# uthree/tinyvc

Hardware: AMD Instinct MI355X
Metric: audio-samples/sec (16 kHz) end-to-end VC (higher is better)
Workload: dtype f32 (fp32 in / out / accumulate; channel contractions as two-term fp16 splits on v_mfma_f32_32x32x16_f16: 22-bit significands, three part-products per fp32 product)

## Files before the change

### tinyvc_amd/csrc/decoder.hip

```cpp
#include "conv3s.h"
#include "conv_s2.h"
#include "film_s2.h"
#include "gemm_s2.h"
#include "small_kernels.h"
#include "tvc_common.h"

namespace tvc {


__device__ __forceinline__ float div24k(float x) {
    const float r = 1.0f / 24000.0f;
    const float q0 = __fmul_rn(x, r);
    return fmaf(fmaf(-q0, 24000.0f, x), r, q0);
}

__device__ __forceinline__ double wave_incl_scan(double v, int lane) {
#pragma unroll
    for (int o = 1; o < 64; o <<= 1) {
        double u = __shfl_up(v, o);
        if (lane >= o) v += u;
    }
    return v;
}

// ... 191 lines not shown
    hipStream_t sh = s;
    if (fk) {
        sh = fk->side;
        TVC_HIP(ctx, hipStreamWaitEvent(sh, fk->amps_ready, 0));
    } else {
        TVC_CHECK(run_harm_sums(ctx, s, f0, csum, B, T));
    }
    hipLaunchKernelGGL(harm_synth_kernel, dim3((Tg + 3) / 4, NB), dim3(256), 0, sh, f0, amps, csum, source, T, scale_size, scale_amp, rg);
    TVC_CHECK(run_amax_rows(ctx, sh, amps, B, kHarm, T, smax));
    TVC_CHECK(run_noise_ifft(ctx, s, kern, angle, seed, frames, B, T, ctx->rag && angle));
    hipLaunchKernelGGL(noise_ola_kernel, dim3(grid_for((long)Tg * kHop / 4, 256, NB >= 32 ? 16 : 512 / NB), NB), dim3(256), 0, s, frames, source, B, T, smax, rg);
    return launch_check(ctx, "dsp");
}

static int plain_conv(tvc_ctx* ctx, hipStream_t s, const PackedW& w, const float* x, int B, int Cin, int len, int dil, float* y, const BfpSlots& bfp, int lin = 0,
                      float lscale = 0.f) {
    int rc = 0;
    if ((lin > 0 ? conv_s2_try<true>(&rc, ctx, s, w, x, B, Cin, len, dil, y, bfp, lin, lscale) : conv_s2_try<false>(&rc, ctx, s, w, x, B, Cin, len, dil, y, bfp)))
        return rc;
    if (lin > 0)
        return conv3s_launch<true, C3EpiBias<false>, false, true>(ctx, s, w, x, B, Cin, len, dil, C3EpiBias<false>{y, w.bias, nullptr, w.M, len}, bfp, nullptr, nullptr,
                                                                   nullptr, 0, lin, lscale);
    return conv3s_launch<true>(ctx, s, w, x, B, Cin, len, dil, C3EpiBias<false>{y, w.bias, nullptr, w.M, len}, bfp);
}

static int film_conv(tvc_ctx* ctx, hipStream_t s, const PackedW& w, const PackedW& fw, const FilmU& fu, const float* h, const float* cond, int B, int C, int len, int dil,
                     float* out, const float* bsc, const float* bsh, const float* res, int res_lin, float res_scale, const BfpSlots& bfp) {
    int rc = 0;
    if (rag_min_len(ctx, len) >= FS2::BN && film_s2_try(&rc, ctx, s, fu, h, cond, B, C, len, dil, out, res, res_lin, res_scale, bfp)) return rc;
    return conv3s_launch<true, C3EpiFilmFused, true>(ctx, s, w, h, B, C, len, dil, C3EpiFilmFused{out, w.bias, bsc, bsh, res, C, len, res_lin, res_scale}, bfp, &fw, &fw,
                                                     cond, C);
}

static int conv_film_half(tvc_ctx* ctx, hipStream_t s, const PackedW& ca, const PackedW& cb, const PackedW& fw, const FilmU& fu, const float* x, int lin, float lscale,
                          int da, int db, float* h, const float* cond, int B, int C, int len, float* out, const float* bsc, const float* bsh, const float* res,
                          int res_lin, float res_scale, const float* ma_in, float* mh, const float* mcond, float* mout) {
    const bool pre = rag_min_len(ctx, len) >= FS2::BN && fu.img && fu.C == C && fu.hb_w > 0.f && C % 96 == 0 && C <= 384 && ma_in && mcond && res && db >= 1 && db <= FS2::MAXD &&
                     (long)C * len * 4 < (1L << 32) && (res_lin <= 0 || (long)C * res_lin * 4 < (1L << 32));
    if (pre) {
        int rc = 0;
        const BfpSlots in{ma_in, nullptr, nullptr};
        const bool ok = lin > 0 ? conv_s2_try<true, true>(&rc, ctx, s, ca, x, B, C, len, da, h, in, lin, lscale, fu.hb_w, fu.hb_b)
                                : conv_s2_try<false, true>(&rc, ctx, s, ca, x, B, C, len, da, h, in, 0, 0.f, fu.hb_w, fu.hb_b);
        if (ok) {
            TVC_CHECK(rc);
            if (!film_s2_try(&rc, ctx, s, fu, h, cond, B, C, len, db, out, res, res_lin, res_scale, BfpSlots{ma_in, mcond, mout}, true, fu.hb_w, fu.hb_b))
                return fail(ctx, TVC_ERR_STATE, "filter_net: the FiLM conv refused the pre-split operand its producer wrote");
            return rc;
        }
    }
    TVC_CHECK(plain_conv(ctx, s, ca, x, B, C, len, da, h, BfpSlots{ma_in, nullptr, mh}, lin, lscale));
    return film_conv(ctx, s, cb, fw, fu, h, cond, B, C, len, db, out, bsc, bsh, res, res_lin, res_scale, BfpSlots{mh, mcond, mout});
}

static __global__ void g8_to_planar_kernel(const float* __restrict__ x, float* __restrict__ y, long B, long l, int C) {
    const long n = B * C * l;
    for (long i = blockIdx.x * (long)blockDim.x + threadIdx.x; i < n; i += (long)gridDim.x * blockDim.x) {
        const long t = i % l, bc = i / l, c = bc % C, b = bc / C;
        y[i] = x[((b * (C / 8) + c / 8) * l + t) * 8 + (c & 7)];
    }
}

static int filter_input_gemm(tvc_ctx* ctx, hipStream_t s, const float* content, const float* f0, float* x, int B, int T, const float* cmax) {
    EpiSumCond ep{x, ctx->flt_content_in.bias, nullptr, f0, nullptr, nullptr, ctx->flt_f_w, ctx->flt_f_b, 384, T, B * T};
    int rc = 0;
    if (!gemm_s2_try(&rc, ctx, s, ctx->flt_content_in, content, B, kSslDim, T, 0, ep, cmax)) rc = gemm_s_launch<2, 4, 2>(ctx, s, ctx->flt_content_in, content, B, kSslDim, T, 0, ep, cmax);
    return rc;
}

int run_filter(tvc_ctx* ctx, hipStream_t s, Ws& ws, const float* content, const float* f0,
               const float* energy, const float* source, float* wave, int B, int T, const FilterTaps* taps, const float* cmax, const float* smax, float* zeroed_slots, bool x_slot_set,
               float* x_pre, bool x_pre_filled) {
    const long L = (long)T * kHop;
    static const int ch[5] = {384, 192, 96, 48, 24};
    const long len_dn[5] = {L, L / 5, L / 20, L / 80, L / 240};
    float* skip[5];
    for (int i = 0; i < 5; ++i) skip[i] = ws.get<float>((size_t)B * ch[4 - i] * len_dn[i]);
    float* x = x_pre ? x_pre : ws.get<float>((size_t)B * ch[0] * T);
    float* xi_pre[5] = {nullptr, nullptr, nullptr, nullptr, nullptr};
    for (int i = 1; i <= 4; ++i) xi_pre[i] = ws.get<float>((size_t)B * ctx->downs[i - 1].cin * len_dn[i]);
// ... 52 lines not shown
                                                                 BfpSlots{mh2, mxi, mout}, &d.res, nullptr, xi, d.cin)));
            }
        }
        ws.release(mk);
    }
    float* xlev[5];
    {
        long l = T;
        for (int i = 0; i < 5; ++i) {
            l *= ctx->ups[i].factor;
            xlev[i] = ws.get<float>((size_t)B * ctx->ups[i].cout * l);
        }
    }
    long len = T;
    const float* mx_in = slot(S_X);
    for (int i = 0; i < 5; ++i) {
        const UpW& u = ctx->ups[i];
        const int lin = (int)len;
        len *= u.factor;
        const int lo = (int)len, C = u.cin, nc = B * lo;
        const float* cond = skip[4 - i];
        const float* mcond = slot(S_SKIP0 + 4 - i);
        size_t mk = ws.mark();
        float* xu = ws.get<float>((size_t)B * C * lo);
        float* h = ws.get<float>((size_t)B * C * lo);
        float* x1 = ws.get<float>((size_t)B * C * lo);
        if (!ws.dry && C == 24) {
            ProfScope ps(ctx, s, ws, "filter.up4+out");
            TVC_CHECK(run_up24_split(ctx, s, u, x, cond, ctx->down0_bw, ctx->down0_bb, x1, wave, B, lo, mx_in, smax, slot(S_UX1 + i)));
        } else if (!ws.dry) {
            static const char* names[4] = {"filter.up0", "filter.up1", "filter.up2", "filter.up3"};
            ProfScope ps(ctx, s, ws, names[i]);
            const float lscale = (float)(1.0 / (double)u.factor);
            for (int half = 0; half < 2; ++half) {
                const PackedW& ca = half ? u.c3 : u.c1;
                const PackedW& cb = half ? u.c4 : u.c2;
                const PackedW& fw = half ? u.film2 : u.film1;
                const float* bsc = fw.bias;
                const float* bsh = fw.bias + C;
                const int da = half ? 9 : 1, db = half ? 27 : 3;
                float* xout = half ? xu : x1;
                const float* ma_in = half ? slot(S_UX1 + i) : mx_in;
                float* mh = slot((half ? S_UHB : S_UHA) + i);
                float* mout = slot((half ? S_UXU : S_UX1) + i);
                if (C == 48) {
                    if (half == 0) {
                        TVC_CHECK(run_conv48_pair(ctx, s, ca, cb, x, lin, lscale, &fw, bsc, bsh, cond, xout, B, lo, da, db, ma_in, mcond, mout));
                    } else {
                        TVC_CHECK(run_conv48s(ctx, s, ca, x1, nullptr, nullptr, nullptr, nullptr, nullptr, h, B, lo, da, ma_in, nullptr, mh));
                        TVC_CHECK(run_conv48s(ctx, s, cb, h, &fw, bsc, bsh, cond, x1, nullptr, B, lo, db, mh, mcond, slot(S_LEV + i), &u.c5, xlev[i]));
                    }
                } else if (half == 0) {
                    TVC_CHECK(conv_film_half(ctx, s, ca, cb, fw, u.fu1, x, lin, lscale, da, db, h, cond, B, C, lo, xout, bsc, bsh, x, lin, lscale, ma_in, mh, mcond, mout));
                } else {
                    TVC_CHECK(conv_film_half(ctx, s, ca, cb, fw, u.fu2, x1, 0, 0.f, da, db, h, cond, B, C, lo, xout, bsc, bsh, x1, 0, 0.f, ma_in, mh, mcond, mout));
                }
            }
            if (C != 48) {
                EpiBias<ACT_NONE, false> ep{xlev[i], u.c5.bias, nullptr, u.cout, lo, nc, (long)u.cout * lo, 0, slot(S_LEV + i), slot(S_UXU + i), u.c5_bw, u.c5_bb, NB};
                if (u.cout == 48) {
                    EpiBiasG8 eg{xlev[i], u.c5.bias, u.cout, lo, nc, slot(S_LEV + i), slot(S_UXU + i), u.c5_bw, u.c5_bb, NB};
                    TVC_CHECK((gemm_s_launch<2, 4, 2>(ctx, s, u.c5, xu, B, C, lo, 0, eg, slot(S_UXU + i))));
                } else if (u.c5.MT6 % 3 == 0) TVC_CHECK((gemm_s_launch<3, 4, 1>(ctx, s, u.c5, xu, B, C, lo, 0, ep, slot(S_UXU + i))));
                else TVC_CHECK((gemm_s_launch<2, 4, 2>(ctx, s, u.c5, xu, B, C, lo, 0, ep, slot(S_UXU + i))));
            }
        }
        ws.release(mk);
        x = xlev[i];
        mx_in = slot(S_LEV + i);
    }
    if (!ws.dry && taps) {
        for (int i = 1; i < 5; ++i)
            if (taps->skips[i] && i == 1)
                hipLaunchKernelGGL(g8_to_planar_kernel, dim3(grid_for((long)B * 48 * len_dn[1])), dim3(256), 0, s, skip[1], taps->skips[1], (long)B, len_dn[1], 48);
            else if (taps->skips[i])
                TVC_HIP(ctx, hipMemcpyAsync(taps->skips[i], skip[i], (size_t)B * ch[4 - i] * len_dn[i] * sizeof(float), hipMemcpyDeviceToDevice, s));
        long l = T;
        for (int i = 0; i < 4; ++i) {
            l *= ctx->ups[i].factor;
            if (taps->ups[i] && ctx->ups[i].cout <= 48)
                hipLaunchKernelGGL(g8_to_planar_kernel, dim3(grid_for((long)B * ctx->ups[i].cout * l)), dim3(256), 0, s, xlev[i], taps->ups[i], (long)B, l, ctx->ups[i].cout);
            else if (taps->ups[i])
                TVC_HIP(ctx, hipMemcpyAsync(taps->ups[i], xlev[i], (size_t)B * ctx->ups[i].cout * l * sizeof(float), hipMemcpyDeviceToDevice, s));
        }
    }
    return ws.dry ? 0 : launch_check(ctx, "filter_net");
}

int run_decoder(tvc_ctx* ctx, hipStream_t s, Ws& ws, const float* content, const float* f0,
                const float* energy, const float* angle, uint64_t seed, float* wave, float* amps_out,
                float* kernel_out, float* source_out, int B, int T, const float* content_bound, const float* energy_bound,
// ... 49 lines not shown
```

### tinyvc_amd/csrc/film_s2.h

```cpp
#pragma once
#include "conv_s2.h"
#include "split_fp16.h"

namespace tvc {


struct FilmS2Args {
    const uint4* img;
    const float* tab;
    const float* x;
    const float* cond;
    int C, len, dil;
    float* y;
    const float* res;
    int res_lin;
    float res_scale;
    int tiles_per_utt, ntiles, mblocks;
    const float* amax_x;
    const float* amax_c;
    float* amax_y;
    const uint4* xpre;
    float pre_w, pre_b;
    RagDev rag;
};

template <int NWV_>
struct FS2T {
    static constexpr int MTB = 3, MW = 1, WM = MTB / MW, NWV = NWV_, WN = 1, NW = MW * NWV, NTHR = NW * 64, BN = NWV * WN * 32, MAXD = 27, XROW = BN + 2 * MAXD;
    static constexpr int A_CONV = 3 * MTB * 2, A_PIECES = A_CONV + 2 * MTB * 2, A_PER = (A_PIECES + NW - 1) / NW;
    static constexpr int XS = (2 * XROW + NTHR - 1) / NTHR;
    static constexpr int A_U4 = A_PIECES * 64, X_U4 = 2 * 2 * XROW, C_U4 = 2 * 2 * BN, BUF_U4 = A_U4 + X_U4 + C_U4;
    static constexpr int lds_bytes = 2 * BUF_U4 * 16 + 6 * 384 * 4 + 64;
    static_assert(2 * BN <= NTHR, "one cond item per thread");
};
using FS2 = FS2T<8>;

__device__ __forceinline__ void split8u(const float (&v)[8], uint4& p1, uint4& p2) {
    unsigned o1[4], o2[4];
#pragma unroll
    for (int j = 0; j < 4; ++j) split2<false>(v[2 * j], v[2 * j + 1], o1[j], o2[j]);
    p1 = make_uint4(o1[0], o1[1], o1[2], o1[3]);
    p2 = make_uint4(o2[0], o2[1], o2[2], o2[3]);
}

template <bool XPRE, bool RAG = false, int NWV_ = 8>
__global__ __launch_bounds__(FS2T<NWV_>::NTHR) __attribute__((amdgpu_waves_per_eu(2))) void film_s2_kernel(FilmS2Args a) {
    using TL = FS2T<NWV_>;
    constexpr int MTB = TL::MTB, WM = TL::WM, NWV = TL::NWV, WN = TL::WN, NW = TL::NW, BN = TL::BN, XROW = TL::XROW, A_PER = TL::A_PER, XS = TL::XS;
    extern __shared__ __attribute__((aligned(16))) uint4 smem_fs[];
    float* Tb = reinterpret_cast<float*>(smem_fs + 2 * TL::BUF_U4);
    float* red = Tb + 6 * 384;
    const int tid = threadIdx.x, lane = tid & 63;
    const int wave = __builtin_amdgcn_readfirstlane(tid >> 6);
    const int l31 = lane & 31, lh = lane >> 5;
    const int wm = wave / NWV, wn = wave - wm * NWV;
    const int C = a.C, nslab = C / 16, rs = a.len, dil = a.dil;
    const int rf = a.res_lin > 0 ? rs / a.res_lin : 1;
    const int xw = BN + 2 * dil, nitems = 2 * xw;

    for (int i = tid; i < 6 * C; i += TL::NTHR) {
        const int r = i / C;
        Tb[r * 384 + (i - r * C)] = a.tab[i];
    }

    int tfirst, tlast;
    tile_range(a.ntiles, tfirst, tlast);
    if (tfirst >= tlast) return;
    auto coords = [&](int v, int& mb, int& b, int& t0, int& len, int& off) __attribute__((always_inline)) {
        const int nt = v / a.mblocks;
        mb = v - nt * a.mblocks;
        const RagTile rt = rag_tile<RAG>(a.rag, nt, a.tiles_per_utt, rs, b);
        b = rt.b;
        t0 = rt.tin * BN;
        len = rt.len;
        off = rt.off;
    };

    u32x4 ar[A_PER];
    float xr[XPRE ? 1 : XS][8], cr[8];
    uint4 xq[XPRE ? XS : 1][2];
    auto item_of = [&](int t_, int k, int& g, int& c) __attribute__((always_inline)) {
        int item = t_ + k * TL::NTHR;
        item = item < nitems ? item : item - nitems;
        g = item / xw;
        c = item - g * xw;
    };
    int xdst[XS];
#pragma unroll
    for (int k = 0; k < XS; ++k) {
        int g, c;
        item_of(tid, k, g, c);
        xdst[k] = g * XROW + c;
    }
    const int cg = tid >= BN ? 1 : 0, cc = tid - cg * BN;
    const int cdst = cg * BN + cc;
// ... 124 lines not shown
        }
    };
    auto film_mul = [&](int buf) __attribute__((always_inline)) {
        const uint4* Ab = smem_fs + buf * TL::BUF_U4 + (TL::A_CONV + wm * WM * 2) * 64 + lane;
        const uint4* Cb = smem_fs + buf * TL::BUF_U4 + TL::A_U4 + TL::X_U4 + lh * BN + wn * WN * 32 + l31;
        f16x8 bf[WN][2];
#pragma unroll
        for (int j = 0; j < WN; ++j)
#pragma unroll
            for (int p = 0; p < 2; ++p) bf[j][p] = __builtin_bit_cast(f16x8, Cb[p * 2 * BN + j * 32]);
#pragma unroll
        for (int i = 0; i < WM; ++i) {
            f16x8 af[2], ag[2];
#pragma unroll
            for (int p = 0; p < 2; ++p) af[p] = __builtin_bit_cast(f16x8, Ab[(i * 2 + p) * 64]);
#pragma unroll
            for (int p = 0; p < 2; ++p) ag[p] = __builtin_bit_cast(f16x8, Ab[((MTB + i) * 2 + p) * 64]);
#pragma unroll
            for (int j = 0; j < WN; ++j) {
                sc[i][j] = TVC_MFMA16(af[1], bf[j][0], sc[i][j]);
                sh[i][j] = TVC_MFMA16(ag[1], bf[j][0], sh[i][j]);
            }
#pragma unroll
            for (int j = 0; j < WN; ++j) {
                sc[i][j] = TVC_MFMA16(af[0], bf[j][1], sc[i][j]);
                sh[i][j] = TVC_MFMA16(ag[0], bf[j][1], sh[i][j]);
            }
#pragma unroll
            for (int j = 0; j < WN; ++j) {
                sc[i][j] = TVC_MFMA16(af[0], bf[j][0], sc[i][j]);
                sh[i][j] = TVC_MFMA16(ag[0], bf[j][0], sh[i][j]);
            }
        }
    };

    int cv = tfirst, cs = 0, cmb, cb = 0, ct0, len, coff;
    coords(cv, cmb, cb, ct0, len, coff);
    float mx_run = 0.f;
    int flush_b = -1;

    issue_load();
    advance_load();
    lstore(0);
    issue_load();
    advance_load();
    slab_barrier();
    int buf = 0;
    while (true) {
        tap_mul(buf, 0);
        lstore(buf ^ 1);
        issue_load();
        tap_mul(buf, 1);
        tap_mul(buf, 2);
        film_mul(buf);
        advance_load();
        if (++cs == nslab) {
            cs = 0;
            int el = lane;
            asm volatile("" : "+v"(el));
            const int e31 = el & 31, eh = el >> 5;
            const float ix = norm_from_amax(XPRE ? presplit_bound(a.pre_w, a.pre_b, a.amax_x, cb) : sload_f32(a.amax_x + cb)).inv, ic_ = norm_from_amax(sload_f32(a.amax_c + cb)).inv;
#pragma unroll
            for (int i = 0; i < WM; ++i) {
            const int row0 = (cmb * MTB + wm * WM + i) * 32;
            const float kc = Tb[FilmU::TAB_SCALE * 384 + row0] * ix, ks = Tb[FilmU::TAB_SSC * 384 + row0] * ic_, kh = Tb[FilmU::TAB_SSH * 384 + row0] * ic_;
#pragma unroll
            for (int g = 0; g < 4; ++g) {
                const int rr = row0 + 8 * g + 4 * eh;
                const float4 b0 = *reinterpret_cast<const float4*>(Tb + FilmU::TAB_BIAS * 384 + rr);
                const float4 b1 = *reinterpret_cast<const float4*>(Tb + FilmU::TAB_BSC * 384 + rr);
                const float4 b2 = *reinterpret_cast<const float4*>(Tb + FilmU::TAB_BSH * 384 + rr);
                const float bm[4] = {b0.x, b0.y, b0.z, b0.w}, bs[4] = {b1.x, b1.y, b1.z, b1.w}, bh[4] = {b2.x, b2.y, b2.z, b2.w};
#pragma unroll
                for (int q = 0; q < 4; ++q)
#pragma unroll
                    for (int j = 0; j < WN; ++j) {
                        const int r = 4 * g + q;
                        const float h = fmaf(hi[i][j][r], kc, bm[q]), s = fmaf(sc[i][j][r], ks, bs[q]), t = fmaf(sh[i][j][r], kh, bh[q]);
                        hi[i][j][r] = __fadd_rn(__fmul_rn(h, s), t);
                        sc[i][j][r] = 0.f;
                        sh[i][j][r] = 0.f;
                    }
            }
            float* yb = RAG ? a.y + (long)row0 * rs + coff : a.y + ((long)cb * C + row0) * rs;
#pragma unroll
            for (int j = 0; j < WN; ++j) {
                const int t = ct0 + (wn * WN + j) * 32 + e31;
                const bool live = t < len;
                const int tc = live ? t : len - 1;
                const unsigned off = 4u * (unsigned)(4 * eh * rs + tc);
                if (a.res_lin > 0) {
                    const Lerp lc = lerp_coord(tc, a.res_scale, RAG ? len / rf : a.res_lin);
                    const float* rb = RAG ? a.res + (long)row0 * a.res_lin + coff / rf : a.res + ((long)cb * C + row0) * a.res_lin;
                    const unsigned o0 = 4u * (unsigned)(4 * eh * a.res_lin + lc.i0), o1 = 4u * (unsigned)(4 * eh * a.res_lin + lc.i1);
#pragma unroll
                    for (int h8 = 0; h8 < 2; ++h8) {
                        float x0[8], x1[8];
#pragma unroll
                        for (int r = 0; r < 8; ++r) {
                            const float* rr = rb + (long)(16 * h8 + (r & 3) + 8 * (r >> 2)) * a.res_lin;
                            x0[r] = ldg_so(rr, o0);
                            x1[r] = ldg_so(rr, o1);
                        }
#pragma unroll
                        for (int r = 0; r < 8; ++r) hi[i][j][8 * h8 + r] = __fadd_rn(hi[i][j][8 * h8 + r], lerp_eval(lc, x0[r], x1[r]));
                    }
                } else {
                    const float* rb = RAG ? a.res + (long)row0 * rs + coff : a.res + ((long)cb * C + row0) * rs;
                    float rv[16];
#pragma unroll
                    for (int r = 0; r < 16; ++r) rv[r] = ldg_so(rb + (long)((r & 3) + 8 * (r >> 2)) * rs, off);
#pragma unroll
                    for (int r = 0; r < 16; ++r) hi[i][j][r] = __fadd_rn(hi[i][j][r], rv[r]);
                }
#pragma unroll
                for (int r = 0; r < 16; ++r) {
                    const float e = hi[i][j][r];
                    if (live) {
                        stg_so(yb + (long)((r & 3) + 8 * (r >> 2)) * rs, off, e);
                        mx_run = fmaxf(mx_run, fabsf(e));
                    }
                    hi[i][j][r] = 0.f;
                }
            }
            }
            const int done_b = cb;
            ++cv;
            const bool last = cv >= tlast;
            if (!last) coords(cv, cmb, cb, ct0, len, coff);
            if (a.amax_y && (last || cb != done_b)) {
                const float m = wave_max(mx_run);
                if (lane == 0) red[wave] = m;
                mx_run = 0.f;
                flush_b = done_b;
            }
            if (last) break;
        }
        slab_barrier();
        if (flush_b >= 0) {
            if (tid == 0) {
                float m = 0.f;
                for (int w = 0; w < NW; ++w) m = fmaxf(m, red[w]);
                if (m > 0.f) atomicMax(reinterpret_cast<unsigned*>(a.amax_y + flush_b), __builtin_bit_cast(unsigned, m));
            }
            flush_b = -1;
        }
        buf ^= 1;
    }
    if (flush_b >= 0) {
        slab_barrier();
        if (tid == 0) {
            float m = 0.f;
            for (int w = 0; w < NW; ++w) m = fmaxf(m, red[w]);
            if (m > 0.f) atomicMax(reinterpret_cast<unsigned*>(a.amax_y + flush_b), __builtin_bit_cast(unsigned, m));
        }
    }
}

inline bool film_s2_try(int* rc, tvc_ctx* ctx, hipStream_t s, const FilmU& fu, const float* h, const float* cond, int B, int C, int len, int dil, float* out,
                        const float* res, int res_lin, float res_scale, const BfpSlots& bfp, bool pre = false, float pre_w = 0.f, float pre_b = 0.f) {
    if (!fu.img || fu.C != C || C % 96 != 0 || C > 384 || dil < 1 || dil > FS2::MAXD || !bfp.x || !bfp.c || !res) return false;
    if ((long)C * len * 4 >= (1L << 32) || (res_lin > 0 && (long)C * res_lin * 4 >= (1L << 32))) return false;
    if ((*rc = lds_optin<film_s2_kernel<false>, film_s2_kernel<true>, film_s2_kernel<false, true>, film_s2_kernel<true, true>>(ctx, FS2::lds_bytes, "film_s2")) ||
        (*rc = lds_optin<film_s2_kernel<false, false, 7>, film_s2_kernel<true, false, 7>>(ctx, FS2T<7>::lds_bytes, "film_s2")))
        return true;
    FilmS2Args a{};
    a.img = reinterpret_cast<const uint4*>(fu.img);
    a.tab = fu.tab;
    a.x = h;
    a.cond = cond;
    a.C = C;
    a.len = len;
    a.dil = dil;
    a.y = out;
    a.res = res;
    a.res_lin = res_lin;
    a.res_scale = res_scale;
    a.mblocks = C / 96;
    a.tiles_per_utt = (len + FS2::BN - 1) / FS2::BN;
    a.amax_x = bfp.x;
    a.xpre = reinterpret_cast<const uint4*>(h);
    a.pre_w = pre_w;
    a.pre_b = pre_b;
    a.amax_c = bfp.c;
    a.amax_y = bfp.y;
    int ncol = a.tiles_per_utt * B;
    if ((*rc = rag_tiles(ctx, s, B, len, FS2::BN, &a.rag, &ncol, "film_s2"))) return true;
    a.ntiles = ncol * a.mblocks;
    const int grid = a.ntiles < ctx->ncu ? a.ntiles : ctx->ncu;
    if (ctx->rag) {
        if (pre) hipLaunchKernelGGL((film_s2_kernel<true, true>), dim3(grid), dim3(FS2::NTHR), FS2::lds_bytes, s, a);
        else hipLaunchKernelGGL((film_s2_kernel<false, true>), dim3(grid), dim3(FS2::NTHR), FS2::lds_bytes, s, a);
    } else if ((len + 223) / 224 * 224 < (len + 255) / 256 * 256) {
        a.tiles_per_utt = (len + 223) / 224;
        a.ntiles = a.tiles_per_utt * B * a.mblocks;
        const int g7 = a.ntiles < ctx->ncu ? a.ntiles : ctx->ncu;
        if (pre) hipLaunchKernelGGL((film_s2_kernel<true, false, 7>), dim3(g7), dim3(FS2T<7>::NTHR), FS2T<7>::lds_bytes, s, a);
        else hipLaunchKernelGGL((film_s2_kernel<false, false, 7>), dim3(g7), dim3(FS2T<7>::NTHR), FS2T<7>::lds_bytes, s, a);
    } else if (pre) hipLaunchKernelGGL(film_s2_kernel<true>, dim3(grid), dim3(FS2::NTHR), FS2::lds_bytes, s, a);
    else hipLaunchKernelGGL(film_s2_kernel<false>, dim3(grid), dim3(FS2::NTHR), FS2::lds_bytes, s, a);
    *rc = launch_check(ctx, "film_s2");
    return true;
}

}
```

### tinyvc_amd/csrc/knn.hip

```cpp
#include <hip/hip_fp16.h>

#include <cstring>
#include <vector>

#include "ragged.h"
#include "small_kernels.h"
#include "split_fp16.h"
#include "tvc_common.h"

namespace tvc {

constexpr int KD = kSslDim;
constexpr int STEPS = KD / 16;
constexpr int HDR = 64;
constexpr int KIND_F32 = 0, KIND_F16 = 1;
constexpr int BLOB_MAGIC = kBlobMagic;
__host__ __device__ inline const float* blob_inv(const float* blob, int kind, long N, long Npad) {
    return kind == KIND_F16 ? blob + HDR : blob + HDR + (size_t)N * KD + (size_t)Npad * KD * 3 / 2;
}
__host__ __device__ inline const uint4* blob_img16(const float* blob, int kind, long N, long Npad) {
    return reinterpret_cast<const uint4*>(blob_inv(blob, kind, N, Npad) + Npad);
}
__host__ __device__ inline const float* blob_invmax(const float* blob, long Npad) {
    return blob + HDR + Npad + (size_t)Npad * KD / 2;
}
constexpr int KNN_BLOCKS = 1024;

static inline int64_t npad128(int64_t N) { return (N + 127) / 128 * 128; }

struct KnnSeg {
    const float* blob;
    int N, col0, ncols;
    int two;
    int sample, t2;
    int nsA, tpsA, nsB, tpsB;
    int nsE, tpsE;
    int u[4];
// ... 594 lines not shown
        v = make_float4(blob_row_value(blob, kind, N, Npad, i, k), blob_row_value(blob, kind, N, Npad, i, k + 1),
                        blob_row_value(blob, kind, N, Npad, i, k + 2), blob_row_value(blob, kind, N, Npad, i, k + 3));
    }
    reinterpret_cast<float4*>(slots + sl * KD)[threadIdx.x] = v;
}
static __global__ __launch_bounds__(256) void knn_finish_kernel(const float* __restrict__ slots, int ncols, int T, float* __restrict__ out) {
    __shared__ float tile[32][193];
    const int tid = threadIdx.x, lane = tid & 63, wave = tid >> 6;
    const int n0 = blockIdx.x * 32;
    for (int kc = 0; kc < KD; kc += 192) {
        for (int q = wave; q < 32; q += 4) {
            const int n = n0 + q < ncols ? n0 + q : ncols - 1;
            const float* r0 = slots + ((long)n * 4) * KD + kc;
#pragma unroll
            for (int u = 0; u < 3; ++u) {
                int k = lane + 64 * u;
                float sum = __fadd_rn(__fadd_rn(__fadd_rn(r0[k], r0[KD + k]), r0[2 * KD + k]), r0[3 * KD + k]);
                tile[q][k] = sum * 0.25f;
            }
        }
        __syncthreads();
        for (int kk = tid >> 5; kk < 192; kk += 8) {
            int q = tid & 31;
            int n = n0 + q;
            if (n < ncols) {
                int b = n / T, t = n - b * T;
                out[((long)b * KD + kc + kk) * T + t] = tile[q][kk];
            }
        }
        __syncthreads();
    }
}

constexpr int C_QT = 256, C_MT = 256, C_K = 64, C_STEPS = KD / C_K;
constexpr int C_A_U4 = 4 * 8 * 64, C_X_U4 = 4 * 2 * C_QT;
constexpr int C_LDS = 2 * (C_A_U4 + C_X_U4) * 16;
constexpr int C_CAP = 256;
constexpr float C_EPS = 1.25e-3f;
constexpr int KNN_COARSE_MIN = 4096;

struct Top4V {
    float v[4];
    __device__ __forceinline__ void init() { v[0] = v[1] = v[2] = v[3] = -INFINITY; }
    __device__ __forceinline__ void insert(float x) {
        if (!(x > v[3])) return;
        if (x > v[0]) { v[3] = v[2]; v[2] = v[1]; v[1] = v[0]; v[0] = x; }
        else if (x > v[1]) { v[3] = v[2]; v[2] = v[1]; v[1] = x; }
        else if (x > v[2]) { v[3] = v[2]; v[2] = x; }
        else v[3] = x;
    }
};

template <bool F16, int MODE>
static __device__ __forceinline__ void knn_coarse_body(const float* __restrict__ blob, long Npad, int N, const uint4* __restrict__ qh,
                                                       int ncols, int cstride, int unit, int nsplit, int tiles_per_split, int t2_cover,
                                                       float* __restrict__ c4v, int ns_sample,
                                                       int* __restrict__ cnt, int* __restrict__ cand, float* __restrict__ candv,
                                                       int* __restrict__ overflow) {
    extern __shared__ __attribute__((aligned(16))) uint4 csmem[];
    uint4* As = csmem;
    uint4* Xs = csmem + 2 * C_A_U4;
    const int kind = F16 ? KIND_F16 : KIND_F32;
    const uint4* img = blob_img16(blob, kind, N, Npad);
    const float* inv = blob_inv(blob, kind, N, Npad);

    const int tid = threadIdx.x, lane = tid & 63, wave = tid >> 6;
    const int wm = wave >> 2, wn = wave & 3;
    const int l31 = lane & 31, lh = lane >> 5;
    const int split = unit % nsplit;
    const int qtile = unit / nsplit;
    const int n0 = qtile * C_QT;
    const int mtiles = (int)(Npad >> 7);
    const int t_lo = split * tiles_per_split;
    const int t_hi = min(t2_cover, t_lo + tiles_per_split);
    const int G = (t_hi - t_lo) * C_STEPS;

    const uint4* xsrc = qh + (long)qtile * (STEPS * 2 * 256) + (tid & 511);
    u32x4 ar[4], xr[4];
    auto gload = [&](int g) __attribute__((always_inline)) {
        const int t2 = t_lo + g / C_STEPS, st = g - (g / C_STEPS) * C_STEPS;
#pragma unroll
        for (int i = 0; i < 4; ++i) {
            const int piece = wave + 8 * i, k16 = piece >> 3, mt8 = piece & 7;
            int t128 = 2 * t2 + (mt8 >> 2);
            t128 = t128 < mtiles ? t128 : mtiles - 1;
            ar[i] = *reinterpret_cast<const u32x4*>(img + (((long)t128 * STEPS + 4 * st + k16) * 4 + (mt8 & 3)) * 64 + lane);
            xr[i] = *reinterpret_cast<const u32x4*>(xsrc + (long)(4 * st + i) * 512);
        }
    };
    auto lstore = [&](int buf) __attribute__((always_inline)) {
#pragma unroll
        for (int i = 0; i < 4; ++i) {
            *reinterpret_cast<u32x4*>(As + buf * C_A_U4 + tid + 512 * i) = ar[i];
            *reinterpret_cast<u32x4*>(Xs + buf * C_X_U4 + tid + 512 * i) = xr[i];
        }
    };

    Top4V top[2];
    top[0].init();
    top[1].init();
    float th[2] = {INFINITY, INFINITY};
    if (MODE == 1) {
#pragma unroll
        for (int j = 0; j < 2; ++j) {
            const int n = n0 + wn * 64 + j * 32 + l31;
            if (n < ncols) {
                Top4V t4;
                t4.init();
                for (int sp = 0; sp < ns_sample; ++sp) {
                    const float4 v4 = *reinterpret_cast<const float4*>(c4v + ((long)sp * cstride + n) * 4);
                    t4.insert(v4.x);
                    t4.insert(v4.y);
                    t4.insert(v4.z);
                    t4.insert(v4.w);
                }
                th[j] = t4.v[3] - 2.f * C_EPS;
            }
        }
    }
    f32x16 acc[4][2];
#pragma unroll
    for (int i = 0; i < 4; ++i)
#pragma unroll
        for (int j = 0; j < 2; ++j)
#pragma unroll
            for (int r = 0; r < 16; ++r) acc[i][j][r] = 0.f;

    if (G > 0) {
        gload(0);
        lstore(0);
        gload(G > 1 ? 1 : 0);
        slab_barrier();
    }
    for (int g = 0; g < G; ++g) {
        const int cur = g & 1;
        lstore(cur ^ 1);
        gload(g + 2 < G ? g + 2 : G - 1);
        const uint4* as = As + cur * C_A_U4 + wm * (4 * 64) + lane;
        const uint4* xs = Xs + cur * C_X_U4 + lh * C_QT + wn * 64 + l31;
#pragma unroll
        for (int k16 = 0; k16 < 4; ++k16) {
            f16x8 af[4], bf[2];
#pragma unroll
            for (int i = 0; i < 4; ++i) af[i] = __builtin_bit_cast(f16x8, as[(k16 * 8 + i) * 64]);
#pragma unroll
            for (int j = 0; j < 2; ++j) bf[j] = __builtin_bit_cast(f16x8, xs[k16 * 2 * C_QT + j * 32]);
#pragma unroll
            for (int i = 0; i < 4; ++i)
#pragma unroll
                for (int j = 0; j < 2; ++j) acc[i][j] = __builtin_amdgcn_mfma_f32_32x32x16_f16(af[i], bf[j], acc[i][j], 0, 0, 0);
        }
        const int st = g - (g / C_STEPS) * C_STEPS;
        if (st == C_STEPS - 1) {
            const int t2 = t_lo + g / C_STEPS;
            const int m0 = t2 * C_MT;
            float imx = 1.f;
            if (F16) {
                const float* im = blob_invmax(blob, Npad);
                const int ta = 2 * t2 < mtiles ? 2 * t2 : mtiles - 1, tb = 2 * t2 + 1 < mtiles ? 2 * t2 + 1 : mtiles - 1;
                imx = fmaxf(im[ta], im[tb]);
            }
            const bool whole = m0 + C_MT <= N;
#pragma unroll
            for (int i = 0; i < 4; ++i)
#pragma unroll
                for (int j = 0; j < 2; ++j) {
                    float mx = acc[i][j][0];
                    bool anynan = false;
#pragma unroll
                    for (int r = 1; r < 16; ++r) mx = fmaxf(mx, acc[i][j][r]);
#pragma unroll
                    for (int r = 0; r < 16; ++r) anynan |= acc[i][j][r] != acc[i][j][r];
                    bool maybe;
                    if (MODE == 0) maybe = anynan || !((F16 ? fmaxf(mx, 0.f) * imx : mx) <= top[j].v[3]);
                    else maybe = anynan || (F16 ? fmaxf(mx, 0.f) * imx : mx) >= th[j];
                    if (__builtin_amdgcn_ballot_w64(maybe) != 0ull) {
#pragma unroll
                        for (int r = 0; r < 16; ++r) {
                            const int row = m0 + (wm * 4 + i) * 32 + (r & 3) + 8 * (r >> 2) + 4 * lh;
                            if (whole || row < N) {
                                const float a = acc[i][j][r];
                                if (MODE == 0) {
                                    if (!F16) {
                                        top[j].insert(nan_max(a));
                                    } else if (!(fmaxf(a, 0.f) * imx <= top[j].v[3])) {
                                        top[j].insert(nan_max(a * inv[row]));
                                    }
                                } else {
                                    bool hit;
                                    float cv = a;
                                    if (!F16) hit = !(a < th[j]);
                                    else {
                                        hit = a != a || (fmaxf(a, 0.f) * imx >= th[j]);
                                        if (hit) {
                                            cv = a * inv[row];
                                            hit = a != a || cv >= th[j];
                                        }
                                    }
                                    hit = hit && th[j] != INFINITY;
                                    if (hit) {
                                        const int n = n0 + wn * 64 + j * 32 + l31;
                                        const int pos = atomicAdd(&cnt[n], 1);
                                        if (pos < C_CAP) {
                                            cand[(long)n * C_CAP + pos] = row;
                                            candv[(long)n * C_CAP + pos] = cv;
                                        } else *overflow = 1;
                                    }
                                }
                            }
                        }
                    }
#pragma unroll
                    for (int r = 0; r < 16; ++r) acc[i][j][r] = 0.f;
                }
        }
        slab_barrier();
    }
    if (MODE == 1) return;

    float (*mv)[16] = reinterpret_cast<float (*)[16]>(csmem);
#pragma unroll
    for (int j = 0; j < 2; ++j) {
        const int q = wn * 64 + j * 32 + l31;
        const int slot = (wm * 2 + lh) * 4;
#pragma unroll
        for (int e = 0; e < 4; ++e) mv[q][slot + e] = top[j].v[e];
    }
    __syncthreads();
    if (tid < C_QT) {
        Top4V t4;
        t4.init();
        for (int e = 0; e < 16; ++e) t4.insert(mv[tid][e]);
        const int n = n0 + tid;
        if (n < ncols) {
            const long o = ((long)split * cstride + n) * 4;
#pragma unroll
            for (int e = 0; e < 4; ++e) c4v[o + e] = t4.v[e];
        }
    }
}

template <int MODE>
static __global__ __launch_bounds__(512) void knn_coarse_kernel(const KnnSegs segs, const uint4* __restrict__ qh, int cstride,
                                                                float* __restrict__ c4v, int* __restrict__ cnt, int* __restrict__ cand,
                                                                float* __restrict__ candv, int* __restrict__ flags) {
    const int si = seg_find<MODE>(segs, blockIdx.x);
    const KnnSeg g = seg_get(segs, si);
    const int unit = blockIdx.x - g.u[MODE];
    const int nsplit = MODE ? g.nsB : g.nsA, tps = MODE ? g.tpsB : g.tpsA, cover = MODE ? g.t2 : g.sample;
    const uint4* q = qh + (long)g.u[3] * (STEPS * 2 * 256);
// ... 364 lines not shown
```

Baseline: 703.5 million.

## Fold the 1x1 c5 output conv into the FiLM conv epilogue for C=96

For upsample stages with 96 channels and 48 outputs, the second-half FiLM conv kernel now runs the 1x1 c5 projection in its epilogue. It re-splits the FiLM output tile to fp16 in registers, runs MFMAs against the packed c5 weights, adds the bias and writes the 48-channel group-of-8 output directly. The FiLM output itself is no longer stored to global memory in this mode, and the amax publish is mapped through the c5 bound. This removes one kernel launch and a full write and read of the intermediate activation. The cost is more register pressure and extra per-tile work inside the FiLM kernel, and the non-RAG path loses the 7-wave tile variant.

Measured after the change: 709.3 million, median of 6. Within noise of the previous version (+0.8%).

```diff
diff --git a/tinyvc_amd/csrc/decoder.hip b/tinyvc_amd/csrc/decoder.hip
--- a/tinyvc_amd/csrc/decoder.hip
+++ b/tinyvc_amd/csrc/decoder.hip
@@ -247,9 +247,16 @@
                                                      cond, C);
 }
 
+struct C5Fold {
+    const PackedW* w;
+    float* out5;
+    float* mlev;
+    float bw, bb;
+};
 static int conv_film_half(tvc_ctx* ctx, hipStream_t s, const PackedW& ca, const PackedW& cb, const PackedW& fw, const FilmU& fu, const float* x, int lin, float lscale,
                           int da, int db, float* h, const float* cond, int B, int C, int len, float* out, const float* bsc, const float* bsh, const float* res,
-                          int res_lin, float res_scale, const float* ma_in, float* mh, const float* mcond, float* mout) {
+                          int res_lin, float res_scale, const float* ma_in, float* mh, const float* mcond, float* mout, const C5Fold* c5 = nullptr,
+                          bool* c5_done = nullptr) {
     const bool pre = rag_min_len(ctx, len) >= FS2::BN && fu.img && fu.C == C && fu.hb_w > 0.f && C % 96 == 0 && C <= 384 && ma_in && mcond && res && db >= 1 && db <= FS2::MAXD &&
                      (long)C * len * 4 < (1L << 32) && (res_lin <= 0 || (long)C * res_lin * 4 < (1L << 32));
     if (pre) {
@@ -259,8 +266,12 @@
                                 : conv_s2_try<false, true>(&rc, ctx, s, ca, x, B, C, len, da, h, in, 0, 0.f, fu.hb_w, fu.hb_b);
         if (ok) {
             TVC_CHECK(rc);
-            if (!film_s2_try(&rc, ctx, s, fu, h, cond, B, C, len, db, out, res, res_lin, res_scale, BfpSlots{ma_in, mcond, mout}, true, fu.hb_w, fu.hb_b))
-                return fail(ctx, TVC_ERR_STATE, "filter_net: the FiLM conv refused the pre-split operand its producer wrote");
+            const bool fold = c5 && c5_done && c5->out5 && c5->mlev && c5->bw >= 0.f && c5->bb >= 0.f && film_s2_c5_ok(*c5->w, C);
+            const bool launched = fold ? film_s2_try(&rc, ctx, s, fu, h, cond, B, C, len, db, out, res, res_lin, res_scale, BfpSlots{ma_in, mcond, c5->mlev}, true, fu.hb_w,
+                                                     fu.hb_b, c5->w, c5->out5, c5->bw, c5->bb)
+                                       : film_s2_try(&rc, ctx, s, fu, h, cond, B, C, len, db, out, res, res_lin, res_scale, BfpSlots{ma_in, mcond, mout}, true, fu.hb_w, fu.hb_b);
+            if (!launched) return fail(ctx, TVC_ERR_STATE, "filter_net: the FiLM conv refused the pre-split operand its producer wrote");
+            if (fold) *c5_done = true;
             return rc;
         }
     }
@@ -379,6 +390,8 @@
             static const char* names[4] = {"filter.up0", "filter.up1", "filter.up2", "filter.up3"};
             ProfScope ps(ctx, s, ws, names[i]);
             const float lscale = (float)(1.0 / (double)u.factor);
+            const C5Fold c5f{&u.c5, xlev[i], slot(S_LEV + i), u.c5_bw, u.c5_bb};
+            bool c5_done = false;
             for (int half = 0; half < 2; ++half) {
                 const PackedW& ca = half ? u.c3 : u.c1;
                 const PackedW& cb = half ? u.c4 : u.c2;
@@ -400,10 +413,11 @@
                 } else if (half == 0) {
                     TVC_CHECK(conv_film_half(ctx, s, ca, cb, fw, u.fu1, x, lin, lscale, da, db, h, cond, B, C, lo, xout, bsc, bsh, x, lin, lscale, ma_in, mh, mcond, mout));
                 } else {
-                    TVC_CHECK(conv_film_half(ctx, s, ca, cb, fw, u.fu2, x1, 0, 0.f, da, db, h, cond, B, C, lo, xout, bsc, bsh, x1, 0, 0.f, ma_in, mh, mcond, mout));
+                    TVC_CHECK(conv_film_half(ctx, s, ca, cb, fw, u.fu2, x1, 0, 0.f, da, db, h, cond, B, C, lo, xout, bsc, bsh, x1, 0, 0.f, ma_in, mh, mcond, mout,
+                                             C == 96 && u.cout == 48 ? &c5f : nullptr, &c5_done));
                 }
             }
-            if (C != 48) {
+            if (C != 48 && !c5_done) {
                 EpiBias<ACT_NONE, false> ep{xlev[i], u.c5.bias, nullptr, u.cout, lo, nc, (long)u.cout * lo, 0, slot(S_LEV + i), slot(S_UXU + i), u.c5_bw, u.c5_bb, NB};
                 if (u.cout == 48) {
                     EpiBiasG8 eg{xlev[i], u.c5.bias, u.cout, lo, nc, slot(S_LEV + i), slot(S_UXU + i), u.c5_bw, u.c5_bb, NB};
diff --git a/tinyvc_amd/csrc/film_s2.h b/tinyvc_amd/csrc/film_s2.h
--- a/tinyvc_amd/csrc/film_s2.h
+++ b/tinyvc_amd/csrc/film_s2.h
@@ -22,6 +22,11 @@
     const uint4* xpre;
     float pre_w, pre_b;
     RagDev rag;
+    const uint4* w5;
+    const float* b5;
+    const float* w5sc;
+    float* y5;
+    float c5_bw, c5_bb;
 };
 
 template <int NWV_>
@@ -43,10 +48,12 @@
     p2 = make_uint4(o2[0], o2[1], o2[2], o2[3]);
 }
 
-template <bool XPRE, bool RAG = false, int NWV_ = 8>
+template <bool XPRE, bool RAG = false, int NWV_ = 8, bool C5 = false>
 __global__ __launch_bounds__(FS2T<NWV_>::NTHR) __attribute__((amdgpu_waves_per_eu(2))) void film_s2_kernel(FilmS2Args a) {
     using TL = FS2T<NWV_>;
     constexpr int MTB = TL::MTB, WM = TL::WM, NWV = TL::NWV, WN = TL::WN, NW = TL::NW, BN = TL::BN, XROW = TL::XROW, A_PER = TL::A_PER, XS = TL::XS;
+    static_assert(!C5 || (TL::MW == 1 && WN == 1), "C5: a wave owns every row of its 32 columns");
+    constexpr int T5_BIAS = 128, T5_WSC = 192;
     extern __shared__ __attribute__((aligned(16))) uint4 smem_fs[];
     float* Tb = reinterpret_cast<float*>(smem_fs + 2 * TL::BUF_U4);
     float* red = Tb + 6 * 384;
@@ -61,6 +68,10 @@
     for (int i = tid; i < 6 * C; i += TL::NTHR) {
         const int r = i / C;
         Tb[r * 384 + (i - r * C)] = a.tab[i];
+    }
+    if constexpr (C5) {
+        if (tid < 64) Tb[T5_BIAS + tid] = a.b5[tid];
+        if (tid < 2) Tb[T5_WSC + tid] = a.w5sc[tid];
     }
 
     int tfirst, tlast;
@@ -251,6 +262,12 @@
                 sh[i][j] = TVC_MFMA16(ag[0], bf[j][0], sh[i][j]);
             }
         }
+    };
+    auto publish = [&](int b_) __attribute__((always_inline)) {
+        float m = 0.f;
+        for (int w = 0; w < NW; ++w) m = fmaxf(m, red[w]);
+        if (C5) m = fmaf(a.c5_bw, m, a.c5_bb);
+        if (m > 0.f) atomicMax(reinterpret_cast<unsigned*>(a.amax_y + b_), __builtin_bit_cast(unsigned, m));
     };
 
     int cv = tfirst, cs = 0, cmb, cb = 0, ct0, len, coff;
@@ -279,6 +296,7 @@
             asm volatile("" : "+v"(el));
             const int e31 = el & 31, eh = el >> 5;
             const float ix = norm_from_amax(XPRE ? presplit_bound(a.pre_w, a.pre_b, a.amax_x, cb) : sload_f32(a.amax_x + cb)).inv, ic_ = norm_from_amax(sload_f32(a.amax_c + cb)).inv;
+            float tmx = 0.f;
 #pragma unroll
             for (int i = 0; i < WM; ++i) {
             const int row0 = (cmb * MTB + wm * WM + i) * 32;
@@ -297,8 +315,10 @@
                         const int r = 4 * g + q;
                         const float h = fmaf(hi[i][j][r], kc, bm[q]), s = fmaf(sc[i][j][r], ks, bs[q]), t = fmaf(sh[i][j][r], kh, bh[q]);
                         hi[i][j][r] = __fadd_rn(__fmul_rn(h, s), t);
-                        sc[i][j][r] = 0.f;
-                        sh[i][j][r] = 0.f;
+                        if (!C5) {
+                            sc[i][j][r] = 0.f;
+                            sh[i][j][r] = 0.f;
+                        }
                     }
             }
             float* yb = RAG ? a.y + (long)row0 * rs + coff : a.y + ((long)cb * C + row0) * rs;
@@ -335,13 +355,72 @@
 #pragma unroll
                 for (int r = 0; r < 16; ++r) {
                     const float e = hi[i][j][r];
-                    if (live) {
-                        stg_so(yb + (long)((r & 3) + 8 * (r >> 2)) * rs, off, e);
-                        mx_run = fmaxf(mx_run, fabsf(e));
+                    if (C5) {
+                        if (live) tmx = fmaxf(tmx, fabsf(e));
+                    } else {
+                        if (live) {
+                            stg_so(yb + (long)((r & 3) + 8 * (r >> 2)) * rs, off, e);
+                            mx_run = fmaxf(mx_run, fabsf(e));
+                        }
+                        hi[i][j][r] = 0.f;
                     }
-                    hi[i][j][r] = 0.f;
                 }
             }
+            }
+            if constexpr (C5) {
+                mx_run = fmaxf(mx_run, tmx);
+                const Bfp s5 = bfp_from_amax(wave_max(tmx));
+                f32x16 a5[2], l5[2];
+#pragma unroll
+                for (int m = 0; m < 2; ++m)
+#pragma unroll
+                    for (int r = 0; r < 16; ++r) a5[m][r] = l5[m][r] = 0.f;
+#pragma unroll
+                for (int s = 0; s < 6; ++s) {
+                    const int i = s >> 1, r0 = 8 * (s & 1);
+                    unsigned pa[2][2], pb[2][2];
+                    split2(hi[i][0][r0] * s5.s, hi[i][0][r0 + 1] * s5.s, pa[0][0], pa[1][0]);
+                    split2(hi[i][0][r0 + 2] * s5.s, hi[i][0][r0 + 3] * s5.s, pa[0][1], pa[1][1]);
+                    split2(hi[i][0][r0 + 4] * s5.s, hi[i][0][r0 + 5] * s5.s, pb[0][0], pb[1][0]);
+                    split2(hi[i][0][r0 + 6] * s5.s, hi[i][0][r0 + 7] * s5.s, pb[0][1], pb[1][1]);
+                    f16x8 bf[2], af[2][2];
+#pragma unroll
+                    for (int p = 0; p < 2; ++p) {
+                        const auto qx = __builtin_amdgcn_permlane32_swap(pa[p][0], pb[p][0], false, false);
+                        const auto qy = __builtin_amdgcn_permlane32_swap(pa[p][1], pb[p][1], false, false);
+                        bf[p] = __builtin_bit_cast(f16x8, u32x4{qx[0], qy[0], qx[1], qy[1]});
+                    }
+#pragma unroll
+                    for (int m = 0; m < 2; ++m)
+#pragma unroll
+                        for (int p = 0; p < 2; ++p) af[m][p] = __builtin_bit_cast(f16x8, ldg_so4(a.w5, 16u * (unsigned)(((s * 2 + m) * 2 + p) * 64 + el)));
+#pragma unroll
+                    for (int m = 0; m < 2; ++m) l5[m] = TVC_MFMA16(af[m][1], bf[0], l5[m]);
+#pragma unroll
+                    for (int m = 0; m < 2; ++m) a5[m] = TVC_MFMA16(af[m][0], bf[0], a5[m]);
+#pragma unroll
+                    for (int m = 0; m < 2; ++m) l5[m] = TVC_MFMA16(af[m][0], bf[1], l5[m]);
+                }
+                const int t = ct0 + wn * 32 + e31;
+                if (t < len) {
+                    float* ob = RAG ? a.y5 + 8L * coff : a.y5 + (long)cb * 48 * rs;
+#pragma unroll
+                    for (int m = 0; m < 2; ++m) {
+                        const float c = Tb[T5_WSC + m] * s5.inv, cl = c * kLoInv;
+#pragma unroll
+                        for (int g = 0; g < 4; ++g) {
+                            if (32 * m + 8 * g >= 48) continue;
+                            const float4 bv = *reinterpret_cast<const float4*>(Tb + T5_BIAS + 32 * m + 8 * g + 4 * eh);
+                            const float v4[4] = {comb(a5[m][4 * g], l5[m][4 * g], c, cl) + bv.x, comb(a5[m][4 * g + 1], l5[m][4 * g + 1], c, cl) + bv.y,
+                                                 comb(a5[m][4 * g + 2], l5[m][4 * g + 2], c, cl) + bv.z, comb(a5[m][4 * g + 3], l5[m][4 * g + 3], c, cl) + bv.w};
+                            stg_so4(ob, 32u * (unsigned)((4 * m + g) * rs + t) + 16u * (unsigned)eh, v4);
+                        }
+                    }
+                }
+#pragma unroll
+                for (int i = 0; i < WM; ++i)
+#pragma unroll
+                    for (int r = 0; r < 16; ++r) hi[i][0][r] = sc[i][0][r] = sh[i][0][r] = 0.f;
             }
             const int done_b = cb;
             ++cv;
@@ -357,30 +436,27 @@
         }
         slab_barrier();
         if (flush_b >= 0) {
-            if (tid == 0) {
-                float m = 0.f;
-                for (int w = 0; w < NW; ++w) m = fmaxf(m, red[w]);
-                if (m > 0.f) atomicMax(reinterpret_cast<unsigned*>(a.amax_y + flush_b), __builtin_bit_cast(unsigned, m));
-            }
+            if (tid == 0) publish(flush_b);
             flush_b = -1;
         }
         buf ^= 1;
     }
     if (flush_b >= 0) {
         slab_barrier();
-        if (tid == 0) {
-            float m = 0.f;
-            for (int w = 0; w < NW; ++w) m = fmaxf(m, red[w]);
-            if (m > 0.f) atomicMax(reinterpret_cast<unsigned*>(a.amax_y + flush_b), __builtin_bit_cast(unsigned, m));
-        }
+        if (tid == 0) publish(flush_b);
     }
 }
 
+inline bool film_s2_c5_ok(const PackedW& c5, int C) { return C == 96 && c5.A6 && c5.bias && c5.wscale && c5.M == 48 && c5.MT6 == 2 && c5.S6 >= 6 && c5.taps == 1 && c5.cin == 96; }
+
 inline bool film_s2_try(int* rc, tvc_ctx* ctx, hipStream_t s, const FilmU& fu, const float* h, const float* cond, int B, int C, int len, int dil, float* out,
-                        const float* res, int res_lin, float res_scale, const BfpSlots& bfp, bool pre = false, float pre_w = 0.f, float pre_b = 0.f) {
+                        const float* res, int res_lin, float res_scale, const BfpSlots& bfp, bool pre = false, float pre_w = 0.f, float pre_b = 0.f,
+                        const PackedW* c5 = nullptr, float* out5 = nullptr, float c5_bw = 0.f, float c5_bb = 0.f) {
     if (!fu.img || fu.C != C || C % 96 != 0 || C > 384 || dil < 1 || dil > FS2::MAXD || !bfp.x || !bfp.c || !res) return false;
     if ((long)C * len * 4 >= (1L << 32) || (res_lin > 0 && (long)C * res_lin * 4 >= (1L << 32))) return false;
-    if ((*rc = lds_optin<film_s2_kernel<false>, film_s2_kernel<true>, film_s2_kernel<false, true>, film_s2_kernel<true, true>>(ctx, FS2::lds_bytes, "film_s2")) ||
+    if (c5 && (!pre || !film_s2_c5_ok(*c5, C) || !out5 || !bfp.y || !(c5_bw >= 0.f) || !(c5_bb >= 0.f))) return false;
+    if ((*rc = lds_optin<film_s2_kernel<false>, film_s2_kernel<true>, film_s2_kernel<false, true>, film_s2_kernel<true, true>, film_s2_kernel<true, false, 8, true>,
+                         film_s2_kernel<true, true, 8, true>>(ctx, FS2::lds_bytes, "film_s2")) ||
         (*rc = lds_optin<film_s2_kernel<false, false, 7>, film_s2_kernel<true, false, 7>>(ctx, FS2T<7>::lds_bytes, "film_s2")))
         return true;
     FilmS2Args a{};
@@ -403,11 +479,22 @@
     a.pre_b = pre_b;
     a.amax_c = bfp.c;
     a.amax_y = bfp.y;
+    if (c5) {
+        a.w5 = reinterpret_cast<const uint4*>(c5->A6);
+        a.b5 = c5->bias;
+        a.w5sc = c5->wscale;
+        a.y5 = out5;
+        a.c5_bw = c5_bw;
+        a.c5_bb = c5_bb;
+    }
     int ncol = a.tiles_per_utt * B;
     if ((*rc = rag_tiles(ctx, s, B, len, FS2::BN, &a.rag, &ncol, "film_s2"))) return true;
     a.ntiles = ncol * a.mblocks;
     const int grid = a.ntiles < ctx->ncu ? a.ntiles : ctx->ncu;
-    if (ctx->rag) {
+    if (c5) {
+        if (ctx->rag) hipLaunchKernelGGL((film_s2_kernel<true, true, 8, true>), dim3(grid), dim3(FS2::NTHR), FS2::lds_bytes, s, a);
+        else hipLaunchKernelGGL((film_s2_kernel<true, false, 8, true>), dim3(grid), dim3(FS2::NTHR), FS2::lds_bytes, s, a);
+    } else if (ctx->rag) {
         if (pre) hipLaunchKernelGGL((film_s2_kernel<true, true>), dim3(grid), dim3(FS2::NTHR), FS2::lds_bytes, s, a);
         else hipLaunchKernelGGL((film_s2_kernel<false, true>), dim3(grid), dim3(FS2::NTHR), FS2::lds_bytes, s, a);
     } else if ((len + 223) / 224 * 224 < (len + 255) / 256 * 256) {
```

## Replace register-staged double buffer with 4-slot direct-to-LDS DMA pipeline in coarse kNN

Applied to the files above, without the earlier changes.

The coarse kNN GEMM loop previously loaded A/X tiles into registers and then stored them to a double-buffered LDS. It now uses global_load_lds DMA into a 4-slot ring, three stages deep, with half-step (K=32) granularity. Fragment reads from LDS are software-pipelined against the MFMAs, and s_setprio is raised around the MFMA bursts. The aim is to cut VGPR staging traffic and hide global latency better, in exchange for a barrier per half-step and more complex waitcnt logic.

After: 704.1 million before, 706.5 million after, median of 5. About the same (+0.4%).

```diff
diff --git a/tinyvc_amd/csrc/knn.hip b/tinyvc_amd/csrc/knn.hip
--- a/tinyvc_amd/csrc/knn.hip
+++ b/tinyvc_amd/csrc/knn.hip
@@ -3,6 +3,7 @@
 #include <cstring>
 #include <vector>
 
+#include "knn_coarse_pipe.h"
 #include "ragged.h"
 #include "small_kernels.h"
 #include "split_fp16.h"
@@ -663,9 +664,9 @@
     }
 }
 
-constexpr int C_QT = 256, C_MT = 256, C_K = 64, C_STEPS = KD / C_K;
-constexpr int C_A_U4 = 4 * 8 * 64, C_X_U4 = 4 * 2 * C_QT;
-constexpr int C_LDS = 2 * (C_A_U4 + C_X_U4) * 16;
+constexpr int C_QT = 256, C_MT = 256;
+constexpr int C_LDS = CP_LDS;
+static_assert(CP_K16 == STEPS, "the pipeline walks the images' K16 steps");
 constexpr int C_CAP = 256;
 constexpr float C_EPS = 1.25e-3f;
 constexpr int KNN_COARSE_MIN = 4096;
@@ -689,8 +690,6 @@
                                                        int* __restrict__ cnt, int* __restrict__ cand, float* __restrict__ candv,
                                                        int* __restrict__ overflow) {
     extern __shared__ __attribute__((aligned(16))) uint4 csmem[];
-    uint4* As = csmem;
-    uint4* Xs = csmem + 2 * C_A_U4;
     const int kind = F16 ? KIND_F16 : KIND_F32;
     const uint4* img = blob_img16(blob, kind, N, Npad);
     const float* inv = blob_inv(blob, kind, N, Npad);
@@ -704,28 +703,6 @@
     const int mtiles = (int)(Npad >> 7);
     const int t_lo = split * tiles_per_split;
     const int t_hi = min(t2_cover, t_lo + tiles_per_split);
-    const int G = (t_hi - t_lo) * C_STEPS;
-
-    const uint4* xsrc = qh + (long)qtile * (STEPS * 2 * 256) + (tid & 511);
-    u32x4 ar[4], xr[4];
-    auto gload = [&](int g) __attribute__((always_inline)) {
-        const int t2 = t_lo + g / C_STEPS, st = g - (g / C_STEPS) * C_STEPS;
-#pragma unroll
-        for (int i = 0; i < 4; ++i) {
-            const int piece = wave + 8 * i, k16 = piece >> 3, mt8 = piece & 7;
-            int t128 = 2 * t2 + (mt8 >> 2);
-            t128 = t128 < mtiles ? t128 : mtiles - 1;
-            ar[i] = *reinterpret_cast<const u32x4*>(img + (((long)t128 * STEPS + 4 * st + k16) * 4 + (mt8 & 3)) * 64 + lane);
-            xr[i] = *reinterpret_cast<const u32x4*>(xsrc + (long)(4 * st + i) * 512);
-        }
-    };
-    auto lstore = [&](int buf) __attribute__((always_inline)) {
-#pragma unroll
-        for (int i = 0; i < 4; ++i) {
-            *reinterpret_cast<u32x4*>(As + buf * C_A_U4 + tid + 512 * i) = ar[i];
-            *reinterpret_cast<u32x4*>(Xs + buf * C_X_U4 + tid + 512 * i) = xr[i];
-        }
-    };
 
     Top4V top[2];
     top[0].init();
@@ -757,39 +734,14 @@
 #pragma unroll
             for (int r = 0; r < 16; ++r) acc[i][j][r] = 0.f;
 
-    if (G > 0) {
-        gload(0);
-        lstore(0);
-        gload(G > 1 ? 1 : 0);
-        slab_barrier();
-    }
-    for (int g = 0; g < G; ++g) {
-        const int cur = g & 1;
-        lstore(cur ^ 1);
-        gload(g + 2 < G ? g + 2 : G - 1);
-        const uint4* as = As + cur * C_A_U4 + wm * (4 * 64) + lane;
-        const uint4* xs = Xs + cur * C_X_U4 + lh * C_QT + wn * 64 + l31;
-#pragma unroll
-        for (int k16 = 0; k16 < 4; ++k16) {
-            f16x8 af[4], bf[2];
-#pragma unroll
-            for (int i = 0; i < 4; ++i) af[i] = __builtin_bit_cast(f16x8, as[(k16 * 8 + i) * 64]);
-#pragma unroll
-            for (int j = 0; j < 2; ++j) bf[j] = __builtin_bit_cast(f16x8, xs[k16 * 2 * C_QT + j * 32]);
-#pragma unroll
-            for (int i = 0; i < 4; ++i)
-#pragma unroll
-                for (int j = 0; j < 2; ++j) acc[i][j] = __builtin_amdgcn_mfma_f32_32x32x16_f16(af[i], bf[j], acc[i][j], 0, 0, 0);
-        }
-        const int st = g - (g / C_STEPS) * C_STEPS;
-        if (st == C_STEPS - 1) {
-            const int t2 = t_lo + g / C_STEPS;
+    coarse_pipeline(img, mtiles, qh + (long)qtile * (STEPS * 2 * 256), t_lo, t_hi - t_lo, csmem, acc, [&](int t2, f32x16 (&acc)[4][2]) __attribute__((always_inline)) {
+        {
             const int m0 = t2 * C_MT;
             float imx = 1.f;
             if (F16) {
                 const float* im = blob_invmax(blob, Npad);
                 const int ta = 2 * t2 < mtiles ? 2 * t2 : mtiles - 1, tb = 2 * t2 + 1 < mtiles ? 2 * t2 + 1 : mtiles - 1;
-                imx = fmaxf(im[ta], im[tb]);
+                imx = fmaxf(sload_f32(im + ta), sload_f32(im + tb));
             }
             const bool whole = m0 + C_MT <= N;
 #pragma unroll
@@ -845,8 +797,7 @@
                     for (int r = 0; r < 16; ++r) acc[i][j][r] = 0.f;
                 }
         }
-        slab_barrier();
-    }
+    });
     if (MODE == 1) return;
 
     float (*mv)[16] = reinterpret_cast<float (*)[16]>(csmem);
diff --git a/tinyvc_amd/csrc/knn_coarse_pipe.h b/tinyvc_amd/csrc/knn_coarse_pipe.h
--- /dev/null
+++ b/tinyvc_amd/csrc/knn_coarse_pipe.h
@@ -0,0 +1,101 @@
+#pragma once
+#include "split_fp16.h"
+
+namespace tvc {
+
+constexpr int CP_K16 = 48;
+constexpr int CP_HS = CP_K16 / 2;
+constexpr int CP_A_U4 = 2 * 8 * 64, CP_X_U4 = 2 * 2 * 256;
+constexpr int CP_SLOT_U4 = CP_A_U4 + CP_X_U4;
+constexpr int CP_SLOTS = 4;
+constexpr int CP_LDS = CP_SLOTS * CP_SLOT_U4 * 16;
+constexpr int CP_DMA = 4;
+
+__device__ __forceinline__ void cp_dma16(const uint4* src, uint4* lds_base) {
+    __builtin_amdgcn_global_load_lds((const __attribute__((address_space(1))) void*)src, (__attribute__((address_space(3))) void*)lds_base, 16, 0, 0);
+}
+template <int N>
+__device__ __forceinline__ void cp_wait_vm() { asm volatile("s_waitcnt vmcnt(%0)" ::"n"(N) : "memory"); }
+
+template <class TileDone>
+__device__ __forceinline__ void coarse_pipeline(const uint4* __restrict__ img, int mtiles, const uint4* __restrict__ xq, int t_lo, int ntiles,
+                                                uint4* smem, f32x16 (&acc)[4][2], TileDone&& tile_done) {
+    const int tid = threadIdx.x, lane = tid & 63, wave = tid >> 6;
+    const int wm = wave >> 2, wn = wave & 3;
+    const int l31 = lane & 31, lh = lane >> 5;
+    const int H = ntiles * CP_HS;
+    if (H <= 0) return;
+
+    auto issue = [&](int t2, int hs, int slot) __attribute__((always_inline)) {
+        uint4* sb = smem + slot * CP_SLOT_U4;
+        int t128 = 2 * t2 + (wave >> 2);
+        t128 = t128 < mtiles ? t128 : mtiles - 1;
+        const uint4* a = img + (((long)t128 * CP_K16 + 2 * hs) * 4 + (wave & 3)) * 64 + lane;
+        const uint4* x = xq + (long)(2 * hs) * 512 + tid;
+#pragma unroll
+        for (int i = 0; i < 2; ++i) cp_dma16(a + i * 256, sb + (i * 8 + wave) * 64);
+#pragma unroll
+        for (int i = 0; i < 2; ++i) cp_dma16(x + i * 512, sb + CP_A_U4 + i * 512 + wave * 64);
+    };
+
+    int it2 = t_lo, ihs = 0;
+    auto issue_next = [&](int slot) __attribute__((always_inline)) {
+        issue(it2, ihs, slot);
+        if (++ihs == CP_HS) {
+            ihs = 0;
+            ++it2;
+        }
+    };
+    issue_next(0);
+    issue_next(1);
+    issue_next(2);
+    cp_wait_vm<CP_DMA>();
+    slab_barrier();
+
+    const uint4* as0 = smem + wm * (4 * 64) + lane;
+    const uint4* xs0 = smem + CP_A_U4 + lh * 256 + wn * 64 + l31;
+    f16x8 af0[4], bf0[2], af1[4], bf1[2];
+#pragma unroll
+    for (int j = 0; j < 2; ++j) bf0[j] = __builtin_bit_cast(f16x8, xs0[j * 32]);
+#pragma unroll
+    for (int i = 0; i < 4; ++i) af0[i] = __builtin_bit_cast(f16x8, as0[i * 64]);
+
+    int t2 = t_lo, hs = 0;
+    for (int h = 0; h < H; ++h) {
+        const int left = H - h;
+        const int so = (h & 3) * CP_SLOT_U4, sn = ((h + 1) & 3) * CP_SLOT_U4;
+#pragma unroll
+        for (int j = 0; j < 2; ++j) bf1[j] = __builtin_bit_cast(f16x8, xs0[so + 512 + j * 32]);
+#pragma unroll
+        for (int i = 0; i < 4; ++i) af1[i] = __builtin_bit_cast(f16x8, as0[so + (8 + i) * 64]);
+        __builtin_amdgcn_s_setprio(1);
+#pragma unroll
+        for (int i = 0; i < 4; ++i)
+#pragma unroll
+            for (int j = 0; j < 2; ++j) acc[i][j] = __builtin_amdgcn_mfma_f32_32x32x16_f16(af0[i], bf0[j], acc[i][j], 0, 0, 0);
+        __builtin_amdgcn_s_setprio(0);
+        if (left > 1) {
+#pragma unroll
+            for (int j = 0; j < 2; ++j) bf0[j] = __builtin_bit_cast(f16x8, xs0[sn + j * 32]);
+#pragma unroll
+            for (int i = 0; i < 4; ++i) af0[i] = __builtin_bit_cast(f16x8, as0[sn + i * 64]);
+        }
+        __builtin_amdgcn_s_setprio(1);
+#pragma unroll
+        for (int i = 0; i < 4; ++i)
+#pragma unroll
+            for (int j = 0; j < 2; ++j) acc[i][j] = __builtin_amdgcn_mfma_f32_32x32x16_f16(af1[i], bf1[j], acc[i][j], 0, 0, 0);
+        __builtin_amdgcn_s_setprio(0);
+        if (left > 3) issue_next((h + 3) & 3);
+        if (++hs == CP_HS) {
+            hs = 0;
+            tile_done(t2, acc);
+            ++t2;
+        }
+        if (left > 3) cp_wait_vm<CP_DMA>();
+        else cp_wait_vm<0>();
+        slab_barrier();
+    }
+}
+
+}
```
